# NLESC-JCER/Fortran_Davidson

Hardware: AMD Instinct MI355X
Metric: Davidson iterations/sec (dense DPR solve, matrix resident in HBM) + A*V HBM GB/s vs roofline (higher is better)
Workload: dtype f64

## Files before the change

fortran_davidson_amd/csrc/engine.hip:

```cpp
#include "engine_internal.h"

thread_local std::string g_err;
int fail(const std::string& msg) {
  g_err = msg;
  return 1;
}

int bind(E* e) {
  e->h0_take = e->h0_cols;
  e->h0_cols = 0;
  HIPCHK(hipSetDevice(e->device));
  return 0;
}

int collect_events(E* e) {
  e->ev_open = 0;
  for (int i = 0; i < e->ev_used; ++i) {
    if (!e->ev_done[i]) continue;
    HIPCHK(hipEventSynchronize(e->ev[i][1]));
    float ms = 0;
    HIPCHK(hipEventElapsedTime(&ms, e->ev[i][0], e->ev[i][1]));
    if (e->ev_kind[i] == 0) {
      e->st.apply_ms += ms;
      e->st.apply_bytes += e->ev_bytes[i];
// ... 79 lines not shown
    HIPCHK(hipEventSynchronize(b.done));
    b.pending = false;
  }
  std::memset(b.host, 0, sizeof(double) * total);
  size_t off = 0;
  for (int k = 0; k < n; ++k) {
    SmallMat& mt = mats[k];
    double* dst = b.host + off;
    if (mt.image) {
      mt.ldm = pg_image_tiles(mt.q);
      pack_operand_image(mt.src, mt.ld, mt.p, mt.q, dst);
    } else {
      mt.ldm = roundup(std::max(mt.p, 1), 4);
      for (int j = 0; j < mt.q; ++j) std::memcpy(dst + j * mt.ldm, mt.src + j * mt.ld, sizeof(double) * mt.p);
    }
    mt.dev = b.dev + off;
    off += (size_t)pg_image_doubles(mt.p, mt.q);
  }
  HIPCHK(hipMemcpyAsync(b.dev, b.host, sizeof(double) * total, hipMemcpyHostToDevice, e->stream));
  HIPCHK(hipEventRecord(b.done, e->stream));
  b.pending = true;
  return 0;
}

int small_upload(E* e, int i, const double* src, int64_t ld, int p, int q, int64_t* ldm_out) {
  SmallMat m{src, ld, p, q, nullptr, 0, false};
  CHK(small_upload_multi(e, i, &m, 1));
  *ldm_out = m.ldm;
  return 0;
}
int small_upload_image(E* e, int i, const double* src, int64_t ld, int p, int q, int64_t* tp_out) {
  SmallMat m{src, ld, p, q, nullptr, 0, true};
  CHK(small_upload_multi(e, i, &m, 1));
  *tp_out = m.ldm;
  return 0;
}

double* panel_ptr(E* e, int panel, int col) {
  return e->panel[panel] + (int64_t)col * e->ldp;
}
int check_panel(E* e, int panel, int c0, int k) {
  if (panel < 0 || panel > 5 || !e->panel[panel]) return fail("invalid or unallocated panel id");
  if (c0 < 0 || k < 0 || c0 + k > e->cols_alloc) return fail("panel column range out of bounds");
  return 0;
}

extern "C" const char* dav_last_error(void) { return g_err.c_str(); }
extern "C" int dav_version(void) { return DAV_HIP_ABI_VERSION; }


extern "C" int dav_create(dav_handle_t* h, int device, int64_t n, int max_cols, int gev, int rank, int nranks) {
  if (!h || n <= 0 || max_cols <= 0 || nranks <= 0 || rank < 0 || rank >= nranks) return fail("dav_create: bad arguments");
  *h = nullptr;
  int ndev = 0;
  HIPCHK(hipGetDeviceCount(&ndev));
  if (ndev <= 0) return fail("dav_create: no HIP device visible - the HIP path has no CPU fallback");
  if (device < 0 || device >= ndev) return fail("dav_create: device index out of range");
  E* e = new E();
  int rc = create_impl(e, device, n, max_cols, gev, rank, nranks);
  if (rc != 0) {
    std::string msg = g_err;
    dav_destroy(e);
    g_err = msg;
    return rc;
  }
  *h = e;
  return 0;
}

Tune tune_from_env() {
  Tune t;
  auto geti = [](const char* name, int dflt) { const char* ev = getenv(name); return ev && *ev ? atoi(ev) : dflt; };
  t.sym_wide = geti("DAV_SYM_WIDE", t.sym_wide);
  t.sym_wide32 = geti("DAV_SYM_WIDE32", t.sym_wide32);
  t.sym_pair = geti("DAV_SYM_PAIR", t.sym_pair);
  t.sym_quad = geti("DAV_SYM_QUAD", t.sym_quad);
  t.sym_overlap = geti("DAV_SYM_OVERLAP", t.sym_overlap);
  t.sym_r = geti("DAV_SYM_R", t.sym_r);
  t.sym_tall = geti("DAV_SYM_TALL", t.sym_tall);
  t.sym_gen_wide = geti("DAV_SYM_GEN_WIDE", 1);
  t.sym_run = std::max(0, geti("DAV_SYM_RUN", 0));
  t.sym_run9 = std::max(0, geti("DAV_SYM_RUN9", 0));
  t.sym_mfma4 = geti("DAV_SYM_MFMA4", t.sym_mfma4);
  t.mv_target = std::max(0, geti("DAV_MV_TARGET", 0));
  t.mv_nsplit = std::max(0, geti("DAV_MV_NSPLIT", 0));
  t.b_resident = geti("DAV_B_RESIDENT", t.b_resident);
  t.coll_direct = geti("DAV_COLL_DIRECT", t.coll_direct);
  t.pg_pin = geti("DAV_PG_PIN", t.pg_pin);
  t.gram_wgs = geti("DAV_GRAM_WGS", t.gram_wgs);
  gram_set_fuse_chunks(geti("DAV_GRAM_FUSE", 0));
  t.gjd_trace = getenv("DAV_GJD_TRACE") != nullptr;
  t.harness_libm = geti("DAV_HARNESS_LIBM", 0);
  t.no_h0 = geti("DAV_NO_H0", 0);
  t.cheb_fuse = geti("DAV_CHEB_FUSE", t.cheb_fuse);
  t.coll_select = geti("DAV_COLL_SELECT", 1);
  t.coll_trial_corrupt = geti("DAV_COLL_TRIAL_CORRUPT", 0);
  t.coll_forced = getenv("DAV_SYM_OVERLAP") != nullptr || getenv("DAV_COLL_DIRECT") != nullptr;
  return t;
}

namespace {
struct PoolBlock { void* p; size_t bytes; int device; int kind; uint64_t gen; };
struct Pool {
  std::mutex mu;
  std::vector<PoolBlock> live, idle;
  std::vector<std::pair<int, hipStream_t>> streams;
  uint64_t gen = 0;
  int enabled = -1;
  size_t cap_bytes = 0;
  size_t cap_pinned_bytes = 0;
  int destroying = 0;
};
Pool& pool() { static Pool* p = new Pool; return *p; }
constexpr size_t POOL_MIN_BYTES = 64 << 10;

bool pool_enabled(Pool& P) {
  if (P.enabled < 0) {
    const char* v = getenv("DAVIDSON_BUFFER_CACHE");
    P.enabled = (v && atoi(v) == 0) ? 0 : 1;
    const char* mb = getenv("DAVIDSON_BUFFER_CACHE_MB");
    P.cap_bytes = (size_t)(mb && atol(mb) >= 0 ? atol(mb) : 4096) << 20;
    const char* pmb = getenv("DAVIDSON_BUFFER_CACHE_PINNED_MB");
    P.cap_pinned_bytes = (size_t)(pmb && atol(pmb) >= 0 ? atol(pmb) : 256) << 20;
  }
  return P.enabled == 1;
}
void pool_release_block(const PoolBlock& b) { if (b.kind == 0) (void)hipFree(b.p); else (void)hipHostFree(b.p); }
std::vector<PoolBlock> pool_take_idle(Pool& P, uint64_t before) {
  std::vector<PoolBlock> out;
  for (size_t i = 0; i < P.idle.size();)
    if (P.idle[i].gen < before) { out.push_back(P.idle[i]); P.idle[i] = P.idle.back(); P.idle.pop_back(); } else ++i;
  return out;
}
hipError_t pool_get(void** p, size_t bytes, int kind, unsigned flags) {
  Pool& P = pool();
  int device = 0;
  (void)hipGetDevice(&device);
  const bool cached = bytes >= POOL_MIN_BYTES;
  if (cached) {
    std::lock_guard<std::mutex> lk(P.mu);
    if (pool_enabled(P))
      for (size_t i = 0; i < P.idle.size(); ++i)
        if (P.idle[i].bytes == bytes && P.idle[i].kind == kind && (kind != 0 || P.idle[i].device == device)) {
          *p = P.idle[i].p;
          P.live.push_back(P.idle[i]);
          P.idle[i] = P.idle.back();
          P.idle.pop_back();
          return hipSuccess;
        }
  }
  hipError_t r = kind == 0 ? hipMalloc(p, bytes) : hipHostMalloc(p, bytes, flags);
  if (r != hipSuccess) {
    (void)hipGetLastError();
    std::vector<PoolBlock> drop;
    { std::lock_guard<std::mutex> lk(P.mu); drop = pool_take_idle(P, UINT64_MAX); }
    if (!drop.empty()) {
      for (const PoolBlock& b : drop) pool_release_block(b);
      r = kind == 0 ? hipMalloc(p, bytes) : hipHostMalloc(p, bytes, flags);
    }
  }
  if (r == hipSuccess && cached) {
    std::lock_guard<std::mutex> lk(P.mu);
    P.live.push_back(PoolBlock{*p, bytes, device, kind, 0});
  }
  return r;
}
// ... 389 lines not shown
```

fortran_davidson_amd/csrc/engine_apply.hip:

```cpp
#include "engine_internal.h"

bool inner_f32_tiles(E* e, OpDesc& o) {
  if (e->inner_bits != 32 || o.kind != DAV_KIND_DENSE || o.storage != 1 || o.a32_refused) return false;
  if (o.a32_valid) return true;
  const size_t count = (size_t)std::max<int64_t>(e->sym.ntiles, 1) * SYM_TB * SYM_TB;
  if (!o.a32 && pool_malloc(&o.a32, sizeof(float) * count) != hipSuccess) {
    (void)hipGetLastError();
    o.a32 = nullptr;
    o.a32_refused = true;
    return false;
  }
  launch_tiles_to_f32(e->stream, o.a, o.a32, (int64_t)count);
  o.a32_valid = true;
  return true;
}

static double* sym_slab_t(const E* e, const SymLaunch& L) { return e->sym_slab + (int64_t)L.ngroups * L.dstride; }
static void sym_sweep(E* e, const SymLaunch& L, const OpDesc& o, const SymSet& set, const double* xt) {
  if (L.nitems == 0) return;
  const SymPlan* pl = L.plan;
  const void* tiles = L.use32 ? (const void*)o.a32 : (const void*)o.a;
  double *slabD = e->sym_slab, *slabT = sym_slab_t(e, L);
  const int64_t xs = e->xt_group_stride, ds = L.dstride, ts = L.tstride;
  switch (L.family) {
    case SYM_ROW_STORED:
      return launch_matvec_sym(e->stream, o.a, set.row_off, set.items, set.nitems, xt, L.kk, slabD, slabT, L.ngroups, xs, ds, ts);
    case SYM_ROW_GENERATED:
      return launch_matvec_sym_generated(e->stream, op_params(o), e->n, set.items, set.nitems, xt, L.kk, slabD, slabT, L.ngroups, xs, ds, ts);
    case SYM_SUPER:
      return launch_matvec_sym9(e->stream, L.R, o.kind != DAV_KIND_DENSE, tiles, L.use32, set.row_off, o.kind != DAV_KIND_DENSE ? op_params(o) : OpParams{},
                                e->n, e->sym_nb, pl->items, pl->nitems, pl->zslot_begin, xt, L.kk, slabD, slabT, L.nwg, xs, ds, ts, e->tune.sym_mfma4 != 0);
    case SYM_WIDE:
    case SYM_WIDE_F32:
      return launch_matvec_symw(e->stream, L.nbw, L.tall, L.use32, tiles, set.row_off, e->sym_nb, pl->items, pl->nitems, pl->zslot_begin, xt, L.kk, slabD, slabT, L.nwg, xs, ds, ts);
    case SYM_WIDE_GENERATED:
      return launch_matvec_symw_generated(e->stream, op_params(o), e->n, e->sym_nb, pl->items, pl->nitems, pl->zslot_begin, xt, L.kk, slabD, slabT, L.nwg, xs, ds, ts);
  }
}

static void count_apply(E* e, int which, int kk) { if (which == DAV_OP_A) { e->st.applies += 1; e->st.apply_cols += kk; } }

static int pack_operand(E* e, const double* src, int kk, bool gather) {
  launch_pack_xt(e->stream, src, e->ldp, e->nloc, e->nslab, kk, e->xt, e->xt_group_stride, e->row0);
  if (!gather) return 0;
  const int ngroups = (kk + 15) / 16;
  CollGroup grp(e);
  CHK(grp.begin(5, 8.0 * (double)e->nslab * 16 * ngroups * e->nranks));
  for (int g = 0; g < ngroups; ++g)
    CHK(coll_allgather(e, e->xt + g * e->xt_group_stride + e->row0 * 16, e->xt + g * e->xt_group_stride, (size_t)e->nslab * 16));
  return grp.end("all-gather of the new block", e->stream);
}

static void sym_reduce_groups(E* e, const SymLaunch& L, const SymSet& set, const int64_t* owned, double* out, int64_t chunk_rows, bool accumulate) {
  const int64_t total_rows = (int64_t)e->nranks * e->nslab;
  const double* slabT = sym_slab_t(e, L);
  for (int g = 0; g < L.ngroups; ++g) {
    const int kg = std::min(16, L.kk - 16 * g);
    const double *d = e->sym_slab + g * L.dstride, *t = slabT + g * L.tstride;
    double* og = out + (size_t)g * 16 * (size_t)(chunk_rows ? total_rows : e->ldp);
    if (L.plan)
      launch_sym9_reduce(e->stream, d, t, L.plan->row_begin, L.plan->zslot_begin, owned, L.plan->next_owned, L.R, e->sym_nb, e->nloc, kg, og, e->ldp,
                         chunk_rows, total_rows, accumulate);
    else
      launch_sym_reduce(e->stream, d, t, set.row_begin, owned, e->sym_nb, e->nloc, kg, og, e->ldp, chunk_rows, total_rows, accumulate);
  }
}

static int ensure_sym_wpart(E* e) {
  if (e->sym_wpart) return 0;
  HIPCHK(pool_malloc(&e->sym_wpart, sizeof(double) * (size_t)e->nranks * (size_t)e->nslab * 64));
  HIPCHK(pool_malloc(&e->sym_wrecv, sizeof(double) * (size_t)e->nslab * 64));
  return 0;
}

static int sym_scatter_to_panel(E* e, int kk, double* dst, bool accumulate, const char* what, double* h0 = nullptr, size_t h0_count = 0) {
  const size_t wstride = (size_t)e->nranks * (size_t)e->nslab * 16, rstride = (size_t)e->nslab * 16;
  const int ngroups = (kk + 15) / 16;
  CollGroup grp(e);
  CHK(grp.begin(6, 8.0 * (double)e->nslab * kk * e->nranks));
  for (int g = 0; g < ngroups; ++g)
    CHK(coll_reduce_scatter(e, e->sym_wpart + g * wstride, e->sym_wrecv + g * rstride, (size_t)e->nslab * std::min(16, kk - 16 * g)));
  if (h0) CHK(coll_allreduce(e, h0, h0_count));
  CHK(grp.end(what, e->stream));
  for (int g = 0; g < ngroups; ++g)
    launch_chunk_to_panel(e->stream, e->sym_wrecv + g * rstride, e->nslab, e->nloc, e->nloc_pad, std::min(16, kk - 16 * g), dst + (int64_t)(16 * g) * e->ldp, e->ldp, accumulate);
  return 0;
}

static double sym_stored_bytes(const E* e, const OpDesc& o, const SymSet& set, bool partial, bool use32) {
  return o.kind != DAV_KIND_DENSE ? 0.0 : (use32 ? 4.0 : 8.0) * (partial ? (double)set.ntiles * SYM_TB * SYM_TB : 0.5 * (double)e->n * ((double)e->n + 1.0) / e->nranks);
}

static int apply_sym_overlapped(E* e, int which, OpDesc& o, const double* src, int k, double* dst, bool timed, bool inner) {
  const int step = 32;
  const int nchunks = (k + step - 1) / step;
  if (!e->ov_ready) {
    hipStream_t cs = nullptr;
    hipEvent_t evs[8] = {};
    double* bufs[4] = {};
    auto undo = [&]() {
      for (hipEvent_t v : evs) if (v) (void)hipEventDestroy(v);
      for (double* b : bufs) if (b) (void)pool_free(b);
      if (cs) (void)hipStreamDestroy(cs);
    };
    int prio_least = 0, prio_greatest = 0;
    if (hipDeviceGetStreamPriorityRange(&prio_least, &prio_greatest) != hipSuccess) { (void)hipGetLastError(); prio_greatest = 0; }
    bool ok = hipStreamCreateWithPriority(&cs, hipStreamNonBlocking, prio_greatest) == hipSuccess;
    for (int i = 0; ok && i < 8; ++i) ok = hipEventCreateWithFlags(&evs[i], hipEventDisableTiming) == hipSuccess;
    for (int i = 0; ok && i < 2; ++i) {
      ok = pool_malloc(&bufs[i], sizeof(double) * (size_t)e->nranks * (size_t)e->nslab * 32) == hipSuccess &&
           pool_malloc(&bufs[2 + i], sizeof(double) * (size_t)e->nslab * 32) == hipSuccess;
    }
    if (!ok) {
      (void)hipGetLastError();
      undo();
      return 2;
    }
    e->comm_stream = cs;
    for (int i = 0; i < 2; ++i) {
      e->ov_packed[i] = evs[4 * i]; e->ov_gathered[i] = evs[4 * i + 1]; e->ov_reduced[i] = evs[4 * i + 2]; e->ov_scattered[i] = evs[4 * i + 3];
      e->sym_wpart2[i] = bufs[i]; e->sym_wrecv2[i] = bufs[2 + i];
    }
    e->ov_ready = true;
  }
  const int64_t total_rows = (int64_t)e->nranks * e->nslab;
  const bool tt = has_test_transport(e);
  hipStream_t cs = tt ? e->stream : e->comm_stream;
  const SymLaunch wide = sym_launch(e, o, e->sym, step, false);
  if (sym_ensure_slabs(e, (size_t)2 * (size_t)(wide.dstride + wide.tstride) + 1) != 0) return 2;
  int slot = -1;
  const double stored = sym_stored_bytes(e, o, e->sym, false, false);
  if (timed) CHK(timed_begin(e, which == DAV_OP_A ? 0 : 2, stored * nchunks + 16.0 * (double)e->n * k, &slot));
  auto cols = [&](int i) { return std::min(step, k - i * step); };
  auto xt_of = [&](int i) { return e->xt + (size_t)(i & 1) * 2 * e->xt_group_stride; };
  auto pack_and_gather = [&](int i) -> int {
    const int p = i & 1, kk = cols(i), ng = (kk + 15) / 16;
    launch_pack_xt(e->stream, src + (int64_t)i * step * e->ldp, e->ldp, e->nloc, e->nslab, kk, xt_of(i), e->xt_group_stride, e->row0);
    HIPCHK(hipEventRecord(e->ov_packed[p], e->stream));
// ... 506 lines not shown
```

fortran_davidson_amd/csrc/engine_internal.h:

```cpp
#pragma once
#include "davidson_hip_private.h"
#include "kernels.h"
#include "ingest.h"

#include <dlfcn.h>
#include <fcntl.h>
#include <pthread.h>
#include <sys/mman.h>
#include <sys/stat.h>
#include <unistd.h>
#include <rccl/rccl.h>

#include <algorithm>
#include <chrono>
#include <condition_variable>
#include <ctime>
#include <mutex>
#include <cmath>
#include <cstdio>
#include <cstring>
#include <numeric>
#include <string>
#include <thread>
#include <vector>
// ... 84 lines not shown
  const SymPlan* plan = nullptr;
  int nitems = 0;
  int64_t dstride = 0, tstride = 0;
  int gen_evals = 0;
};

struct SparseStore {
  int64_t* rp = nullptr;
  int32_t* col = nullptr;
  double* val = nullptr;
  CsrItem* items = nullptr;
  CsrLong* longs = nullptr;
  double* part = nullptr;
  int nitems = 0, nlong = 0;
  int64_t nnz = 0;
  int64_t nrows = 0;
  int b = 0;
  int64_t grow0 = 0;
  uint64_t* src = nullptr;
  int64_t* doff = nullptr;
  int64_t* dpos = nullptr;
  int64_t gcount = 0;
  int triangle = 0, rowmaj = 0;
  double* bdiag = nullptr;
  bool bdiag_valid = false;
  double* rbound = nullptr;
  bool rbound_valid = false;
  int32_t* dia_off = nullptr;
  double* dia_val = nullptr;
  int dia_nd = 0;
  int64_t dia_ld = 0;
};

struct OpDesc {
  int kind = DAV_KIND_NONE;
  double* a = nullptr;
  uint64_t seed = 0;
  double sparsity = 0;
  int use_diag = 0;
  double diag_val = 0;
  int trig = 0;
  bool harness_libm = false;
  double* e_table = nullptr;
  double* dadd_table = nullptr;
  double* l2_table = nullptr;
  double* diag = nullptr;
  int storage = 0;
  float* a32 = nullptr;
  bool a32_valid = false, a32_refused = false;
  double* res_a = nullptr;
  int64_t res_tiles = 0;
  int res_first = 0;
  bool res_decided = false;
  bool pass_res = false, pass_gen = false;
  SymSet* res = nullptr;
  SymSet* gen = nullptr;
  dav_device_apply_fn dev_fn = nullptr;
  void* dev_ctx = nullptr;
  SparseStore sp;
};

struct SmallBuf {
  double* dev = nullptr;
  double* host = nullptr;
  hipEvent_t done = nullptr;
  bool pending = false;
};

constexpr int N_SMALL = 4;
constexpr int N_EVPAIRS = 64;

struct Tune {
  int sym_wide = 2;
  int sym_wide32 = 1;
  int sym_pair = 1;
  int sym_quad = 1;
  int sym_overlap = 0;
  int sym_r = 0;
  int sym_tall = 1;
  int sym_gen_wide = 1;
  int sym_run = 0;
  int sym_run9 = 0;
  int sym_mfma4 = 1;
  int64_t mv_target = 0;
  int64_t mv_nsplit = 0;
  int gram_wgs = 0;
  int pg_pin = 1;
  int coll_direct = 0;
  int b_resident = 1;
  bool gjd_trace = false;
  int coll_select = 1;
  int coll_trial_corrupt = 0;
  bool coll_forced = false;
  int no_h0 = 0;
  int harness_libm = 0;
  int cheb_fuse = 1;
};
Tune tune_from_env();

enum { COLL_PATH_UNDECIDED = -1, COLL_PATH_PROGRAM_ORDER = 0, COLL_PATH_DIRECT = 1, COLL_PATH_SECOND_STREAM = 2 };
struct CollTrial {
  bool ran = false;
  int selected = COLL_PATH_PROGRAM_ORDER, columns = 0;
  double ms[3] = {0, 0, 0}, ms_max[3] = {0, 0, 0};
  bool valid[3] = {true, false, false}, valid_all[3] = {true, false, false};
  double differing[3] = {0, 0, 0}, maxdiff[3] = {0, 0, 0};
  std::string message[3];
};

enum { GUESS_NONE = 0, GUESS_ONE_SHOT = 1, GUESS_RESULT = 2 };
struct Watchdog;
struct dav_engine {
  Tune tune;
  int device = 0;
  hipStream_t stream = nullptr;
  int64_t n = 0, nslab = 0, nloc = 0, row0 = 0, nloc_pad = 0, ncols_pad = 0;
  int rank = 0, nranks = 1, gev = 0;
  int max_cols = 0, cols_alloc = 0;
  int m = 0;
  char* arena = nullptr;
  char* arena_host = nullptr;
  double* panel[6] = {nullptr, nullptr, nullptr, nullptr, nullptr, nullptr};
  int64_t ldp = 0;
  double* xt = nullptr;
  int64_t xt_group_stride = 0;
  double* scratch = nullptr;
  size_t scratch_doubles = 0;
  double* gram_dev = nullptr;
  double* gram_host = nullptr;
  double* gram_host_dev = nullptr;
  size_t gram_doubles = 0;
  double* gather_dev = nullptr;
  int64_t* idx_dev = nullptr;
  double* norm_partial = nullptr;
  unsigned* counters = nullptr;
  double* gjd_ws = nullptr;
  double* cheb_ws = nullptr;
  int storage = 0;
  int sym_nb = 0;
  SymSet sym;
  double* sym_slab = nullptr;
  size_t sym_slab_doubles = 0;
  bool sym_no_pair = false;
  bool sym_no_quad = false;
  int inner_bits = 64;
  double* sym_wpart = nullptr;
  double* sym_wrecv = nullptr;
  double* coll_stage = nullptr;
  size_t coll_stage_doubles = 0;
  int coll_path = COLL_PATH_PROGRAM_ORDER;
  CollTrial coll_trial;
  Watchdog* wd = nullptr;
  int group_depth = 0;
  bool group_timed = false;
  long iter_hint = -1;
  std::vector<double> agree_words;
  std::vector<double> agreed_inputs;
  double* agree_pin = nullptr;
  double* h0_dev = nullptr;
  double* cb_x = nullptr;
  size_t cb_x_doubles = 0;
  double* h0_host = nullptr;
  int h0_cap = 0, h0_cols = 0, h0_take = 0;
  int h0_kind[2] = {0, 0};
  hipStream_t comm_stream = nullptr;
  bool ov_ready = false;
// ... 157 lines not shown
```

fortran_davidson_amd/csrc/k_matvec_sym9.hip:

```cpp
#include "kernels.h"
#include <cstdlib>
#include <type_traits>

__device__ __forceinline__ const double* sym9_tile(const double* tiles, const int64_t* __restrict__ row_off, int I, int J) {
  return tiles + (row_off[I] + J) * (int64_t)(SYM_TB * SYM_TB);
}

__device__ __forceinline__ double mfma4_f64(double a, double b, double c) { return __builtin_amdgcn_mfma_f64_4x4x4f64(a, b, c, 0, 0, 0); }

template <int R, bool GEN, bool F32, bool M4, int HARN = 0>
__global__ __launch_bounds__(512, 1) void matvec_sym9_kernel(const void* __restrict__ tiles_v, const int64_t* __restrict__ row_off,
                                                             const int* __restrict__ items,
                                                             const int* __restrict__ zslot_begin, const double* __restrict__ xt,
                                                             double* __restrict__ slabD, double* __restrict__ slabT, int kcols,
                                                             int npair, int64_t xt_gstride, int64_t slabD_gstride,
                                                             int64_t slabT_gstride, int nb, OpParams op, int64_t n) {
  const double* tiles = static_cast<const double*>(tiles_v);
  const float* tiles32 = static_cast<const float*>(tiles_v);
  (void)tiles; (void)tiles32;
  constexpr int NCG = 4 / R;
  constexpr int NRS = 2 * R;
  constexpr int BW = 16 * NCG;
  constexpr int UPJ = SYM_TB / BW;
  constexpr int UPS = 64 / BW;
// ... 320 lines not shown
                        double* slabT, int npair, int64_t xt_gstride, int64_t slabD_gstride, int64_t slabT_gstride, bool m4) {
  dim3 grid(nitems * npair), block(512);
#define DAV_SYM9_LAUNCH(RR, GG, FF, MM, ...)                                                                                     \
  hipLaunchKernelGGL((matvec_sym9_kernel<RR, GG, FF, MM, ##__VA_ARGS__>), grid, block, 0, st, tiles, row_off, items_dev, zslot_begin_dev, xt, slabD, slabT, \
                     kcols, npair, xt_gstride, slabD_gstride, slabT_gstride, nb, op, n)
  const bool harness = gen && op.kind == DAV_KIND_HARNESS;
  const bool hsin = harness && op.trig != 0;
  const bool hlibm = harness && op.libm != 0;
  if (R == 4) {
    if (hlibm) DAV_SYM9_LAUNCH(4, true, false, true, 3);
    else if (hsin) DAV_SYM9_LAUNCH(4, true, false, true, 2);
    else if (harness) DAV_SYM9_LAUNCH(4, true, false, true, 1);
    else if (gen) DAV_SYM9_LAUNCH(4, true, false, true);
    else if (tiles_f32) DAV_SYM9_LAUNCH(4, false, true, true);
    else if (m4) DAV_SYM9_LAUNCH(4, false, false, true);
    else DAV_SYM9_LAUNCH(4, false, false, false);
  } else {
    if (hlibm) DAV_SYM9_LAUNCH(2, true, false, false, 3);
    else if (hsin) DAV_SYM9_LAUNCH(2, true, false, false, 2);
    else if (harness) DAV_SYM9_LAUNCH(2, true, false, false, 1);
    else if (gen) DAV_SYM9_LAUNCH(2, true, false, false);
    else if (tiles_f32) DAV_SYM9_LAUNCH(2, false, true, false);
    else DAV_SYM9_LAUNCH(2, false, false, false);
  }
#undef DAV_SYM9_LAUNCH
}

__global__ __launch_bounds__(256) void tiles_to_f32_kernel(const double* __restrict__ src, float* __restrict__ dst, int64_t count4) {
  for (int64_t e = (int64_t)blockIdx.x * 256 + threadIdx.x; e < count4; e += (int64_t)gridDim.x * 256) {
    const f64x2 a = reinterpret_cast<const f64x2*>(src)[2 * e], b = reinterpret_cast<const f64x2*>(src)[2 * e + 1];
    reinterpret_cast<float4*>(dst)[e] = float4{(float)a.x, (float)a.y, (float)b.x, (float)b.y};
  }
}
void launch_tiles_to_f32(hipStream_t st, const double* src, float* dst, int64_t count) {
  hipLaunchKernelGGL(tiles_to_f32_kernel, dim3(256 * 32), dim3(256), 0, st, src, dst, count / 4);
}

__global__ __launch_bounds__(256) void sym9_reduce_kernel(const double* __restrict__ slabD, const double* __restrict__ slabT,
                                                          const int* __restrict__ row_item_begin, const int* __restrict__ zslot_begin,
                                                          const int64_t* __restrict__ owned, const int* __restrict__ next_owned, int R, int nb,
                                                          int nsuper, int64_t nloc, int k, double* __restrict__ dst, int64_t ldd,
                                                          int64_t chunk_rows, int64_t total_rows, int accumulate) {
  const int J = blockIdx.x, col = blockIdx.y, r = threadIdx.x;
  if (col >= k) return;
  double sum = 0.0;
  const int Sown = J / R, sub = J % R;
  for (int it = row_item_begin[Sown]; it < row_item_begin[Sown + 1]; ++it)
    sum += slabD[(((int64_t)it * R + sub) * 16 + col) * SYM_TB + r];
  auto zt = [&](int S) { return slabT[(((int64_t)zslot_begin[S] + J) * 16 + col) * SYM_TB + r]; };
  double s0 = 0.0, s1 = 0.0, s2 = 0.0, s3 = 0.0;
  const int Send = (nb - 1 > J) ? nsuper : 0;
  if (!owned) {
    int S = (J + 1) / R;
    for (; S + 3 < Send; S += 4) { s0 += zt(S); s1 += zt(S + 1); s2 += zt(S + 2); s3 += zt(S + 3); }
    for (; S < Send; ++S) s0 += zt(S);
  } else {
    int S = (J + 1) / R < nsuper ? next_owned[(J + 1) / R] : nsuper;
    while (S < Send) {
      s0 += zt(S); S = next_owned[S + 1];
      if (S >= Send) break;
      s1 += zt(S); S = next_owned[S + 1];
      if (S >= Send) break;
      s2 += zt(S); S = next_owned[S + 1];
      if (S >= Send) break;
      s3 += zt(S); S = next_owned[S + 1];
    }
  }
  sum += (s0 + s1) + (s2 + s3);
  const int64_t row = (int64_t)J * SYM_TB + r;
  if (chunk_rows > 0) {
    if (row < total_rows) dst[(row / chunk_rows) * (chunk_rows * k) + (int64_t)col * chunk_rows + row % chunk_rows] = sum;
  } else {
    dst[(int64_t)col * ldd + row] = row < nloc ? (accumulate ? dst[(int64_t)col * ldd + row] + sum : sum) : 0.0;
  }
}

void launch_sym9_reduce(hipStream_t st, const double* slabD, const double* slabT, const int* row_item_begin_dev,
                        const int* zslot_begin_dev, const int64_t* owned, const int* next_owned, int R, int nb, int64_t nloc, int k, double* dst,
                        int64_t ldd, int64_t chunk_rows, int64_t total_rows, bool accumulate) {
  const int nsuper = (nb + R - 1) / R;
  hipLaunchKernelGGL(sym9_reduce_kernel, dim3(nb, k), dim3(256), 0, st, slabD, slabT, row_item_begin_dev, zslot_begin_dev, owned, next_owned, R,
                     nb, nsuper, nloc, k, dst, ldd, chunk_rows, total_rows, accumulate && chunk_rows == 0 ? 1 : 0);
}
```

fortran_davidson_amd/csrc/kernels.h:

```cpp
#pragma once
#include "common.h"

constexpr int MV_ROWS = 256;
void launch_pack_xt(hipStream_t st, const double* src, int64_t ld, int64_t nloc, int64_t nslab, int k,
                    double* xt, int64_t xt_group_stride, int64_t row_off);
void launch_matvec_dense(hipStream_t st, const double* A, int64_t lda, int64_t nrows_pad, int64_t ncols_pad,
                         const double* xt, int64_t xt_group_stride, int ngroups, double* slab,
                         int nsplit, int jc);
void launch_matvec_free(hipStream_t st, OpParams op, int64_t row0, int64_t nloc, int64_t n,
                        int64_t nrows_pad, int64_t ncols_pad, const double* xt, int64_t xt_group_stride,
                        int ngroups, double* slab, int nsplit, int jc);
void launch_slab_reduce(hipStream_t st, const double* slab, int nsplit, int64_t nrows_pad, int ngroups,
                        int64_t nloc, int k, double* dst, int64_t ldd);
size_t matvec_slab_doubles(int64_t nrows_pad, int ngroups, int nsplit);
void matvec_plan(int64_t nrows_pad, int64_t ncols_pad, int ngroups, int* nsplit, int* jc, int64_t target = 0, int64_t forced_nsplit = 0);

constexpr int GRAM_MIN_ROWS = 256;
constexpr int GRAM_FUSE_CHUNKS = 24;
constexpr int GRAM_MAX_COUNTERS = 256;
void launch_gram(hipStream_t st, const double* P, int64_t ldp, int p, const double* Q, int64_t ldq, int q,
                 int64_t nrows_pad, double* scratch, double* out_dev, unsigned* counters = nullptr, int wg_target = 0);
size_t gram_scratch_doubles(int p, int q, int64_t nrows_pad);
void gram_set_fuse_chunks(int n);
void launch_gram_multi(hipStream_t st, const double* P, int64_t ldp, int p, const double* const* Qs, int nq, int qeach, int64_t ldq,
                       int64_t nrows_pad, double* scratch, double* out_dev, unsigned* counters = nullptr, int wg_target = 0);

struct PanelGemmArgs {
  const double* P1; int64_t ld1; int p1; const double* M1; int64_t tp1;
  const double* P2; int64_t ld2; int p2; const double* M2; int64_t tp2;
  double* out; int64_t ldo; int q;
  int64_t nloc, nrows_pad;
  int epilogue;
  const double* theta; const double* dA; const double* dB;
  int nnorm; double* norm_partial;
  double* norm_out; unsigned* counter;
  int pin;
  int batch; int64_t batch_stride;
};
static inline int64_t pg_image_tiles(int q) { return ((int64_t)(q > 0 ? q : 1) + 63) / 64 * 4; }
static inline int64_t pg_image_doubles(int p, int q) { return ((int64_t)(p > 0 ? p : 1) + 3) / 4 * pg_image_tiles(q) * 64; }
static inline int64_t pg_image_index(int i, int j, int64_t tp) { return (((int64_t)(i >> 2) * tp + (j >> 4)) << 6) + (j & 15) + 16 * (i & 3); }
constexpr int PG_ROWS = 128;
constexpr int PG_FUSE_BLOCKS = 48;
constexpr int PG_INPLACE_COLS = 64;
void launch_panel_gemm(hipStream_t st, const PanelGemmArgs& a);
void launch_norm_finish(hipStream_t st, const double* partial, int nblocks, int nnorm, double* out);

void launch_generate_dense(hipStream_t st, double* A, int64_t lda, int64_t nrows_pad, int64_t ncols_pad,
                           int64_t row0, int64_t nloc, int64_t n, uint64_t seed, double sparsity,
                           int use_diag, double diag_val);
void launch_diag_dense(hipStream_t st, const double* A, int64_t lda, int64_t row0, int64_t nloc, double* diag);
void launch_diag_free(hipStream_t st, OpParams op, int64_t row0, int64_t nloc, double* diag);
void launch_gather_columns(hipStream_t st, const double* A, int64_t lda, int64_t nrows_pad,
                           const int64_t* idx_dev, int k, double* dst, int64_t ldd);
void launch_unit_columns(hipStream_t st, const int64_t* idx_dev, int k, int64_t row0, int64_t nloc,
                         int64_t nrows_pad, double* dst, int64_t ldd);
void launch_copy_columns(hipStream_t st, const double* src, int64_t lds, double* dst, int64_t ldd,
                         int64_t nrows_pad, int k);
void launch_stream(hipStream_t st, int mode, double* a, const double* b, const double* c, double s, int64_t n);
void launch_harness_rate(hipStream_t st, double* out, int wgs, int iters);
void launch_compare_blocks(hipStream_t st, const double* a, const double* b, int64_t ld, int64_t rows, int k, double* out);
void launch_poke(hipStream_t st, double* p, double delta);
void launch_sum_parts(hipStream_t st, const double* own, const double* stage, int nparts, int self, size_t count, double* out);



void launch_rows_scatter(hipStream_t st, const double* stage, int64_t ldr, int64_t grow0, int64_t nrows, int64_t n,
                         double* dst, int64_t lda, int64_t slab_row0, int64_t slab_rows, int sym, const int64_t* row_off);

struct LincombArgs {
  const double* in[4]; const double* coef; int ldc; int nterms;
  double* out; int64_t ld; int64_t nrows_pad; int m;
};
void launch_lincomb(hipStream_t st, const LincombArgs& a);
void launch_precond(hipStream_t st, const double* in, double* out, int64_t ld, int64_t nloc, int64_t nrows_pad, int m,
                    const double* theta, const double* dA, const double* dB, const double* active);
struct DotsArgs {
  const double* a[4]; const double* b[4]; int npairs; int64_t ld; int64_t nrows_pad; int m; double* partial;
};
int coldots_blocks(int64_t nrows_pad);
void launch_coldots(hipStream_t st, const DotsArgs& a);

constexpr int SYM_TB = 256;
void launch_matvec_sym(hipStream_t st, const double* tiles, const int64_t* row_off, const int* items_dev, int nitems, const double* xt, int kcols,
                       double* slabD, double* slabT, int npair, int64_t xt_gstride, int64_t slabD_gstride, int64_t slabT_gstride);
void launch_matvec_sym_generated(hipStream_t st, OpParams op, int64_t n, const int* items_dev, int nitems, const double* xt, int kcols,
                                 double* slabD, double* slabT, int npair, int64_t xt_gstride, int64_t slabD_gstride,
                                 int64_t slabT_gstride);
void launch_sym_reduce(hipStream_t st, const double* slabD, const double* slabT, const int* row_item_begin_dev, const int64_t* owned,
                       int nb, int64_t nloc, int k, double* dst, int64_t ldd, int64_t chunk_rows, int64_t total_rows, bool accumulate = false);
void launch_matvec_sym9(hipStream_t st, int R, bool gen, const void* tiles, bool tiles_f32, const int64_t* row_off, OpParams op, int64_t n,
                        int nb, const int* items_dev, int nitems, const int* zslot_begin_dev, const double* xt, int kcols, double* slabD,
                        double* slabT, int npair, int64_t xt_gstride, int64_t slabD_gstride, int64_t slabT_gstride, bool mfma4 = true);
void launch_matvec_symw(hipStream_t st, int nbw, bool tall, bool tiles_f32, const void* tiles, const int64_t* row_off, int nb, const int* items_dev,
                        int nitems, const int* zslot_begin_dev, const double* xt, int kcols, double* slabD, double* slabT, int nwg,
                        int64_t xt_gstride, int64_t slabD_gstride, int64_t slabT_gstride);
void launch_matvec_symw_generated(hipStream_t st, OpParams op, int64_t n, int nb, const int* items_dev, int nitems, const int* zslot_begin_dev,
                                  const double* xt, int kcols, double* slabD, double* slabT, int nwg, int64_t xt_gstride, int64_t slabD_gstride,
                                  int64_t slabT_gstride);
void launch_tiles_to_f32(hipStream_t st, const double* src, float* dst, int64_t count);
void launch_sym9_reduce(hipStream_t st, const double* slabD, const double* slabT, const int* row_item_begin_dev,
                        const int* zslot_begin_dev, const int64_t* owned, const int* next_owned, int R, int nb, int64_t nloc, int k, double* dst,
                        int64_t ldd, int64_t chunk_rows, int64_t total_rows, bool accumulate = false);
void launch_generate_sym_tiles(hipStream_t st, double* tiles, const int64_t* row_off_host, int nb, int64_t n, uint64_t seed,
                               double sparsity, int use_diag, double diag_val);
void launch_retile_panel(hipStream_t st, const double* panel, int64_t ldp, int64_t nrows, int ncols, int J, int nb,
                         const int64_t* row_off, double* tiles);
void launch_diag_sym(hipStream_t st, const double* tiles, const int64_t* row_off, int64_t n, int64_t nrows, double* diag);
void launch_gather_columns_sym_rs(hipStream_t st, const double* tiles, const int64_t* row_off, int64_t n, int64_t chunk_rows,
                                  int64_t total_rows, const int64_t* idx_dev, int k, double* dst);
void launch_entries_sym(hipStream_t st, const double* tiles, const int64_t* row_off, const int64_t* idx_dev, int k, double* h0);
void launch_zero_pad_rows(hipStream_t st, double* dst, int64_t ldd, int64_t nloc, int64_t nrows_pad, int k);
void launch_entries_free(hipStream_t st, OpParams op, const int64_t* idx_dev, int k, double* h0);
void launch_entries_dense(hipStream_t st, const double* A, int64_t lda, const int64_t* idx_dev, int k, double* h0);
void launch_gather_columns_free(hipStream_t st, OpParams op, int64_t row0, int64_t nloc, int64_t nrows_pad, const int64_t* idx_dev, int k,
                                double* dst, int64_t ldd);
void launch_gather_columns_sym(hipStream_t st, const double* tiles, const int64_t* row_off, int64_t n, int64_t nrows_pad,
                               const int64_t* idx_dev, int k, double* dst, int64_t ldd);
void launch_chunk_to_panel(hipStream_t st, const double* src, int64_t lds, int64_t nloc, int64_t nrows_pad, int k, double* dst, int64_t ldd,
                           bool accumulate = false);

constexpr int CSR_ROWS = 16;
constexpr int64_t CSR_CHUNK = 1024;
struct CsrItem { int64_t p0, p1; int32_t row, nrows, slot, pad; };
struct CsrLong { int32_t row, first, count, pad; };
void launch_spmm_csr(hipStream_t st, const CsrItem* items, int nitems, const int64_t* rp, const int32_t* col, const double* val,
                     const double* xt, int64_t xt_gstride, int groups, int kk, double* part, double* dst, int64_t ldd);
void launch_spmm_csr_finish(hipStream_t st, const CsrLong* longs, int nlong, const double* part, int kk, double* dst, int64_t ldd);
struct ChebEpi { const double *z, *r, *zprev, *hdr, *ab, *pi; int64_t ld; };
void launch_spmm_csr_cheb(hipStream_t st, const CsrItem* items, int nitems, const int64_t* rp, const int32_t* col, const double* val,
                          const double* xt, int64_t xt_gstride, int groups, int kk, double* part, double* dst, int64_t ldd, const ChebEpi& epi);
void launch_spmm_csr_finish_cheb(hipStream_t st, const CsrLong* longs, int nlong, const double* part, int kk, double* dst, int64_t ldd,
                                 const ChebEpi& epi);

void launch_dia_mark(hipStream_t st, const void* row_ptr, int rp64, const void* col_idx, int ci64, int64_t n, int64_t nnz, int base, int lower,
                     uint8_t* marks, unsigned long long* ndiag);
int64_t dia_leading_dimension(int64_t nloc);
void launch_dia_fill(hipStream_t st, const int64_t* rp, const int32_t* col, const double* val, int64_t nloc, int64_t row0, const int32_t* off,
                     int nd, double* dval, int64_t ld);
void launch_spmm_dia(hipStream_t st, const int32_t* off, int nd, const double* dval, int64_t ld, int64_t nloc, int64_t row0, int64_t n,
                     const double* xt, int64_t xt_gstride, int groups, int kk, double* dst, int64_t ldd);
void launch_spmm_dia_cheb(hipStream_t st, const int32_t* off, int nd, const double* dval, int64_t ld, int64_t nloc, int64_t row0, int64_t n,
                          const double* xt, int64_t xt_gstride, int groups, int kk, double* dst, int64_t ldd, const ChebEpi& epi);

template <class F> void cb_dispatch(int rp64, int ci64, F&& f) {
  if (rp64) {
    if (ci64) f(int64_t{}, int64_t{});
    else f(int64_t{}, int32_t{});
  } else {
    if (ci64) f(int32_t{}, int64_t{});
    else f(int32_t{}, int32_t{});
  }
}

void launch_csr_build_rows(hipStream_t st, const void* rp, int rp64, int64_t n, unsigned long long* info);
void launch_csr_build_check(hipStream_t st, const void* rp, int rp64, const void* col, int ci64, int64_t n, int64_t nnz, int base, int lower,
                            int64_t r0, int64_t nloc, unsigned long long* first_bad, int32_t* mcount, uint32_t* dcount,
                            unsigned long long* dfirst);
void launch_csr_build_locate(hipStream_t st, const void* rp, int rp64, const void* col, int ci64, int64_t n, int base, int64_t p, int64_t* out);
void launch_csr_build_offsets(hipStream_t st, const void* rp, int rp64, int64_t r0, int64_t nloc, const int32_t* mcount, int64_t* lrp,
                              int64_t* tile_sums);
int64_t csr_build_scan_tiles(int64_t m);
void launch_csr_build_scan(hipStream_t st, int64_t* x, int64_t m, int64_t* tile_sums);
void launch_csr_build_scatter(hipStream_t st, const void* rp, int rp64, const void* col, int ci64, const double* vals, int64_t n, int64_t p_lo,
                              int64_t p_hi, int base, int lower, int64_t r0, int64_t nloc, const int64_t* lrp, int32_t* fill, int32_t* ocol,
                              double* oval, uint32_t* tie);
void launch_csr_build_scatter(hipStream_t st, const void* rp, int rp64, const void* col, int ci64, int64_t n, int64_t p_lo, int64_t p_hi,
                              int base, int lower, int64_t r0, int64_t nloc, const int64_t* lrp, int32_t* fill, int32_t* ocol, uint64_t* osrc,
                              uint32_t* tie);
void launch_csr_build_flag(hipStream_t st, const int64_t* lrp, int64_t nloc, int64_t lnnz, const int32_t* ocol, const uint32_t* tie,
                           uint8_t* flag);
template <class V>
void launch_csr_build_sort_rows(hipStream_t st, const int64_t* lrp, int64_t nloc, const uint8_t* flag, int32_t* ocol, V* oval,
                                const uint32_t* tie);
int64_t csr_build_sort_tile();
template <class V>
void launch_csr_build_sort_long(hipStream_t st, int64_t a, int64_t m, int32_t* ocol, V* oval, const uint32_t* tie, uint64_t* k0, V* v0,
                                uint64_t* k1, V* v1);
void launch_csr_build_diag(hipStream_t st, const void* rp, int rp64, const void* col, int ci64, const double* vals, int64_t n, int base,
                           const uint32_t* dcount, const unsigned long long* dfirst, double* diag);

void launch_bsr_build_gather(hipStream_t st, int bs, const uint64_t* src, int64_t lnnzb, const double* vals, int rowmaj, double* val);
void launch_bsr_build_diag(hipStream_t st, int bs, const void* rp, int rp64, const void* col, int ci64, const double* vals, int64_t nb,
                           int base, const uint32_t* dcount, const unsigned long long* dfirst, double* diag);

void launch_sparse_refresh_csr(hipStream_t st, const uint64_t* src, int64_t lnnz, const double* vals, double* val);
// ... 54 lines not shown
```

Measured before the change: 22.68.

## Add single-launch streaming reduce for sym9 slabs across all column groups

Adds a new sym9 reduce kernel that handles every 16-column group in one launch, splitting work into 8-column parts per tile row. It uses nontemporal vectorised f64x2 loads with 4-way unrolled accumulation over the diagonal and transposed slab images, plus vector stores when alignment allows. It becomes the default path (DAV_SYM_REDUCE=1) when a plan exists and the reduce is non-distributed. The aim is to cut per-group launch overhead and raise bandwidth utilisation of the slab reduction, at the cost of a second code path whose indexing must match the existing reduce.

```diff
diff --git a/fortran_davidson_amd/csrc/engine.hip b/fortran_davidson_amd/csrc/engine.hip
--- a/fortran_davidson_amd/csrc/engine.hip
+++ b/fortran_davidson_amd/csrc/engine.hip
@@ -185,6 +185,7 @@
   t.sym_run = std::max(0, geti("DAV_SYM_RUN", 0));
   t.sym_run9 = std::max(0, geti("DAV_SYM_RUN9", 0));
   t.sym_mfma4 = geti("DAV_SYM_MFMA4", t.sym_mfma4);
+  t.sym_reduce = geti("DAV_SYM_REDUCE", t.sym_reduce);
   t.mv_target = std::max(0, geti("DAV_MV_TARGET", 0));
   t.mv_nsplit = std::max(0, geti("DAV_MV_NSPLIT", 0));
   t.b_resident = geti("DAV_B_RESIDENT", t.b_resident);
diff --git a/fortran_davidson_amd/csrc/engine_apply.hip b/fortran_davidson_amd/csrc/engine_apply.hip
--- a/fortran_davidson_amd/csrc/engine_apply.hip
+++ b/fortran_davidson_amd/csrc/engine_apply.hip
@@ -54,6 +54,9 @@
 static void sym_reduce_groups(E* e, const SymLaunch& L, const SymSet& set, const int64_t* owned, double* out, int64_t chunk_rows, bool accumulate) {
   const int64_t total_rows = (int64_t)e->nranks * e->nslab;
   const double* slabT = sym_slab_t(e, L);
+  if (L.plan && !owned && chunk_rows == 0 && e->tune.sym_reduce != 0)
+    return launch_sym9_reduce_stream(e->stream, e->sym_slab, slabT, L.plan->row_begin, L.plan->zslot_begin, L.R, e->sym_nb, e->nloc, L.kk, L.ngroups,
+                                     L.dstride, L.tstride, out, e->ldp, accumulate);
   for (int g = 0; g < L.ngroups; ++g) {
     const int kg = std::min(16, L.kk - 16 * g);
     const double *d = e->sym_slab + g * L.dstride, *t = slabT + g * L.tstride;
diff --git a/fortran_davidson_amd/csrc/engine_internal.h b/fortran_davidson_amd/csrc/engine_internal.h
--- a/fortran_davidson_amd/csrc/engine_internal.h
+++ b/fortran_davidson_amd/csrc/engine_internal.h
@@ -190,6 +190,7 @@
   int sym_run = 0;
   int sym_run9 = 0;
   int sym_mfma4 = 1;
+  int sym_reduce = 1;
   int64_t mv_target = 0;
   int64_t mv_nsplit = 0;
   int gram_wgs = 0;
diff --git a/fortran_davidson_amd/csrc/k_matvec_sym9.hip b/fortran_davidson_amd/csrc/k_matvec_sym9.hip
--- a/fortran_davidson_amd/csrc/k_matvec_sym9.hip
+++ b/fortran_davidson_amd/csrc/k_matvec_sym9.hip
@@ -426,3 +426,120 @@
   hipLaunchKernelGGL(sym9_reduce_kernel, dim3(nb, k), dim3(256), 0, st, slabD, slabT, row_item_begin_dev, zslot_begin_dev, owned, next_owned, R,
                      nb, nsuper, nloc, k, dst, ldd, chunk_rows, total_rows, accumulate && chunk_rows == 0 ? 1 : 0);
 }
+
+constexpr int SRS_NV = 4;
+constexpr int SRS_CW = 2 * SRS_NV;
+constexpr int SRS_PARTS = 16 / SRS_CW;
+constexpr int SRS_PIECE = 2 * 256;
+template <bool FULL>
+__device__ __forceinline__ void sym9_reduce_stream_body(const double* __restrict__ slabD, const double* __restrict__ slabT,
+                                                        const int* __restrict__ row_item_begin, const int* __restrict__ zslot_begin, int R, int nb,
+                                                        int nsuper, int64_t nloc, int k, int ngroups, int64_t dstride, int64_t tstride,
+                                                        double* __restrict__ dst, int64_t ldd, int accumulate, int vec_store) {
+  const int part = blockIdx.x % SRS_PARTS, g = (blockIdx.x / SRS_PARTS) % ngroups, J = (blockIdx.x / SRS_PARTS) / ngroups;
+  const int lane = threadIdx.x;
+  const int col0 = SRS_CW * part + (lane >> 7);
+  const int kg = min(16, k - 16 * g);
+  const int nv = min(SRS_NV, (kg - col0 + 1) / 2);
+  if (nv <= 0) return;
+  const int64_t off = (int64_t)part * SRS_CW * SYM_TB + 2 * lane;
+  const double* D = slabD + g * dstride + off;
+  const double* T = slabT + g * tstride + off;
+  const f64x2 zero = {0.0, 0.0};
+  auto ld = [&](const double* p, int i) { return __builtin_nontemporal_load(reinterpret_cast<const f64x2*>(p + i * SRS_PIECE)); };
+
+  f64x2 sum[SRS_NV], s0[SRS_NV], s1[SRS_NV], s2[SRS_NV], s3[SRS_NV];
+#pragma unroll
+  for (int i = 0; i < SRS_NV; ++i) sum[i] = s0[i] = s1[i] = s2[i] = s3[i] = zero;
+
+  const int Sown = J / R, sub = J % R;
+  const int it_end = row_item_begin[Sown + 1];
+  auto dimg = [&](int it) { return D + ((int64_t)it * R + sub) * 16 * SYM_TB; };
+  int it = row_item_begin[Sown];
+  for (; it + 3 < it_end; it += 4) {
+    f64x2 v[4][SRS_NV];
+#pragma unroll
+    for (int u = 0; u < 4; ++u)
+#pragma unroll
+      for (int i = 0; i < SRS_NV; ++i) v[u][i] = (FULL || i < nv) ? ld(dimg(it + u), i) : zero;
+#pragma unroll
+    for (int u = 0; u < 4; ++u)
+#pragma unroll
+      for (int i = 0; i < SRS_NV; ++i) sum[i] += v[u][i];
+  }
+  {
+    const int rem = it_end - it;
+    f64x2 v[3][SRS_NV];
+#pragma unroll
+    for (int u = 0; u < 3; ++u)
+#pragma unroll
+      for (int i = 0; i < SRS_NV; ++i) v[u][i] = (u < rem && (FULL || i < nv)) ? ld(dimg(it + u), i) : zero;
+#pragma unroll
+    for (int u = 0; u < 3; ++u)
+      if (u < rem) {
+#pragma unroll
+        for (int i = 0; i < SRS_NV; ++i) sum[i] += v[u][i];
+      }
+  }
+
+  auto timg = [&](int S) { return T + ((int64_t)zslot_begin[S] + J) * 16 * SYM_TB; };
+  const int Send = (nb - 1 > J) ? nsuper : 0;
+  int S = (J + 1) / R;
+  for (; S + 3 < Send; S += 4) {
+    f64x2 v[4][SRS_NV];
+#pragma unroll
+    for (int u = 0; u < 4; ++u)
+#pragma unroll
+      for (int i = 0; i < SRS_NV; ++i) v[u][i] = (FULL || i < nv) ? ld(timg(S + u), i) : zero;
+#pragma unroll
+    for (int i = 0; i < SRS_NV; ++i) { s0[i] += v[0][i]; s1[i] += v[1][i]; s2[i] += v[2][i]; s3[i] += v[3][i]; }
+  }
+  {
+    const int rem = Send - S;
+    f64x2 v[3][SRS_NV];
+#pragma unroll
+    for (int u = 0; u < 3; ++u)
+#pragma unroll
+      for (int i = 0; i < SRS_NV; ++i) v[u][i] = (u < rem && (FULL || i < nv)) ? ld(timg(S + u), i) : zero;
+#pragma unroll
+    for (int u = 0; u < 3; ++u)
+      if (u < rem) {
+#pragma unroll
+        for (int i = 0; i < SRS_NV; ++i) s0[i] += v[u][i];
+      }
+  }
+
+  const int64_t row = (int64_t)J * SYM_TB + 2 * (lane & 127);
+#pragma unroll
+  for (int i = 0; i < SRS_NV; ++i) {
+    if (!FULL && i >= nv) break;
+    sum[i] += (s0[i] + s1[i]) + (s2[i] + s3[i]);
+    double* p = dst + (int64_t)(16 * g + col0 + 2 * i) * ldd + row;
+    f64x2 w;
+    w.x = row < nloc ? (accumulate ? p[0] + sum[i].x : sum[i].x) : 0.0;
+    w.y = row + 1 < nloc ? (accumulate ? p[1] + sum[i].y : sum[i].y) : 0.0;
+    if (vec_store) *reinterpret_cast<f64x2*>(p) = w;
+    else { p[0] = w.x; p[1] = w.y; }
+  }
+}
+
+__global__ __launch_bounds__(256) void sym9_reduce_stream_kernel(const double* __restrict__ slabD, const double* __restrict__ slabT,
+                                                                 const int* __restrict__ row_item_begin, const int* __restrict__ zslot_begin,
+                                                                 int R, int nb, int nsuper, int64_t nloc, int k, int ngroups, int64_t dstride,
+                                                                 int64_t tstride, double* __restrict__ dst, int64_t ldd, int accumulate,
+                                                                 int vec_store) {
+  const int part = blockIdx.x % SRS_PARTS, g = (blockIdx.x / SRS_PARTS) % ngroups;
+  if (k - 16 * g >= SRS_CW * (part + 1))
+    sym9_reduce_stream_body<true>(slabD, slabT, row_item_begin, zslot_begin, R, nb, nsuper, nloc, k, ngroups, dstride, tstride, dst, ldd, accumulate, vec_store);
+  else
+    sym9_reduce_stream_body<false>(slabD, slabT, row_item_begin, zslot_begin, R, nb, nsuper, nloc, k, ngroups, dstride, tstride, dst, ldd, accumulate, vec_store);
+}
+
+void launch_sym9_reduce_stream(hipStream_t st, const double* slabD, const double* slabT, const int* row_item_begin_dev,
+                               const int* zslot_begin_dev, int R, int nb, int64_t nloc, int k, int ngroups, int64_t dstride, int64_t tstride,
+                               double* dst, int64_t ldd, bool accumulate) {
+  const int nsuper = (nb + R - 1) / R;
+  const int vec_store = ldd % 2 == 0 && reinterpret_cast<uintptr_t>(dst) % 16 == 0;
+  hipLaunchKernelGGL(sym9_reduce_stream_kernel, dim3(SRS_PARTS * ngroups * nb), dim3(256), 0, st, slabD, slabT, row_item_begin_dev, zslot_begin_dev, R, nb,
+                     nsuper, nloc, k, ngroups, dstride, tstride, dst, ldd, accumulate ? 1 : 0, vec_store);
+}
diff --git a/fortran_davidson_amd/csrc/kernels.h b/fortran_davidson_amd/csrc/kernels.h
--- a/fortran_davidson_amd/csrc/kernels.h
+++ b/fortran_davidson_amd/csrc/kernels.h
@@ -102,6 +102,9 @@
 void launch_sym9_reduce(hipStream_t st, const double* slabD, const double* slabT, const int* row_item_begin_dev,
                         const int* zslot_begin_dev, const int64_t* owned, const int* next_owned, int R, int nb, int64_t nloc, int k, double* dst,
                         int64_t ldd, int64_t chunk_rows, int64_t total_rows, bool accumulate = false);
+void launch_sym9_reduce_stream(hipStream_t st, const double* slabD, const double* slabT, const int* row_item_begin_dev,
+                               const int* zslot_begin_dev, int R, int nb, int64_t nloc, int k, int ngroups, int64_t dstride, int64_t tstride,
+                               double* dst, int64_t ldd, bool accumulate = false);
 void launch_generate_sym_tiles(hipStream_t st, double* tiles, const int64_t* row_off_host, int nb, int64_t n, uint64_t seed,
                                double sparsity, int use_diag, double diag_val);
 void launch_retile_panel(hipStream_t st, const double* panel, int64_t ldp, int64_t nrows, int ncols, int J, int nb,
```

After: 22.68, median of 3. No clear change (-0.0%).
